# limeorange1102/multimodal-av-model

Hardware: AMD Instinct MI355X
Metric: utterances/sec (4 s clip, 25 fps 96x96 lip) at batch 64, full training step (higher is better)
Workload: dtype bf16; 1 GPU; BASELINE metric configuration (= configs[3]'s per-GPU batch): batch 64/GPU x 4 s (T_audio 64000, T_enc 199, 100 lip frames 96x96 x 2 speakers), wav2vec2-large + ResNet-18 + fusion BiLSTM + CTC + contrastive, fwd+bwd+Adam, random-init weights; variant=as_executed, global_batch=64, parallelism=dp1, audio_passes=2, wav2vec2_regularizers=hf-defaults (dropout 0.1, LayerDrop 0.1, SpecAugment 0.05)

## Files before the change

include/av_hip.h:

```cpp
#ifndef AV_HIP_H
#define AV_HIP_H
#ifdef __cplusplus
extern "C" {
#endif

#define AV_OK 0
#define AV_ERR_ARG 1
#define AV_ERR_LAUNCH 2

#define AV_F32 0
#define AV_BF16 1

#define AV_A_ROWMAJOR 0
#define AV_A_TRANS 1
#define AV_A_CONV2D 2
#define AV_A_CONV3D1 3
#define AV_B_NK 0
#define AV_B_KN 1
#define AV_ACT_NONE 0
#define AV_ACT_GELU 1
#define AV_ACT_MUL_GELU_GRAD 2
#define AV_ACT_GELU_GF 3
#define AV_ACT_MUL_AUX 4

// ... 61 lines not shown
                     int Tk, int D, long long q_bs, long long q_rs, long long k_bs, long long k_rs, long long v_bs,
                     long long v_rs, long long o_bs, long long o_rs, const int* klen, float scale, float drop_p,
                     unsigned long long drop_seed, unsigned int drop_stream, void* stream);
int av_attention_bwd(const void* q, const void* k, const void* v, const void* o, const void* dout, const float* lse,
                     float* delta_ws, void* dq, void* dk, void* dv, int B, int H, int Tq, int Tk, int D,
                     const long long* strides, const int* klen, float scale, float drop_p, unsigned long long drop_seed,
                     unsigned int drop_stream, void* stream);
int av_attention_dropmask(void* mask, int B, int H, int Tq, int Tk, float drop_p, unsigned long long drop_seed, unsigned int drop_stream,
                          void* stream);
int av_attention_fwd_mask(const void* q, const void* k, const void* v, void* o, float* lse, int dtype, int B, int H, int Tq,
                          int Tk, int D, long long q_bs, long long q_rs, long long k_bs, long long k_rs, long long v_bs,
                          long long v_rs, long long o_bs, long long o_rs, const int* klen, float scale, float drop_p,
                          unsigned long long drop_seed, unsigned int drop_stream, const void* drop_mask, void* stream);
int av_attention_bwd_mask(const void* q, const void* k, const void* v, const void* o, const void* dout, const float* lse,
                          float* delta_ws, void* dq, void* dk, void* dv, int B, int H, int Tq, int Tk, int D,
                          const long long* strides, const int* klen, float scale, float drop_p, unsigned long long drop_seed,
                          unsigned int drop_stream, const void* drop_mask, void* stream);
int av_softmax_rows(const float* s, void* p, int pdt, long long rows, int cols, float scale, const int* klen,
                    int rows_per_batch, int ld, void* stream);
int av_softmax_bwd_rows(const void* p, int pdt, const float* dp, void* ds, int dsdt, long long rows, int cols,
                        float scale, int ld, void* stream);

int av_conv0_ln_gelu(const float* wav, const float* w, const float* bias, const float* gamma, const float* beta, void* out,
                     int out_dtype, int B, int T_in, int L_out, int C, int k, int stride, float eps, void* stream);

int av_lstm_fwd_step(const float* gx, const void* whh, void* hseq, float* cseq, void* gates, void* out_bt, int dtype,
                     int T, int B, int H, int s, void* stream);
int av_lstm_bwd_step(const void* dout, int dout_dtype, long long do_bs, long long do_ts, void* dgates, const void* whhT,
                     const void* gates, const float* cseq, float* dc, int dtype, int T, int B, int H, int s, void* stream);

#define AV_LSTM_COUNTER_INTS 1024
int av_lstm_fwd_layer(const float* gx, const void* whh, void* hseq, float* cseq, void* gates, void* out_bt, int* counters,
                      int T, int B, int H, void* stream);
int av_lstm_bwd_layer(const void* dout, int dout_dtype, long long do_bs, long long do_ts, void* dgates, const void* whhT,
                      const void* gates, const float* cseq, float* dc, int* counters, int T, int B, int H, void* stream);

int av_mask_downsample(const long long* mask, long long* out, int B, int Tin, int Tout, void* stream);
int av_fusion_gather_lerp_fwd(const float* feat, const long long* mask, int* ws_i32, float* out, long long* mask_out,
                              long long* lens, int B, int Ta, int Tv, int D, int groups, void* stream);
int av_fusion_gather_lerp_bwd(const float* dout, const int* ws_i32, float* dfeat, int B, int Ta, int Tv, int D, int groups,
                              void* stream);
int av_permute_bt(const void* in, int idt, void* out, int odt, int B, int T, int D, void* stream);
int av_gather_rows(const void* src, int sdt, const long long* idx, void* out, int odt, long long n, int D, void* stream);
int av_scatter_rows(const float* src, const long long* idx, float* out, long long n, int D, float alpha, int accumulate,
                    void* stream);
int av_class_order(const long long* mask, long long n, long long* order, void* stream);

int av_conv3d_front(const float* x, const void* w, void* y, float* stats, int B, int T, int H, int W, void* stream);
int av_conv3d_front_pool(const float* x, const void* w, void* ymax, void* ymin, float* stats, int B, int T, int H, int W, void* stream);
int av_bn_prelu_minmax(const void* ymax, const void* ymin, const float* scale, const float* shift, const float* slope, void* out, long long n,
                       void* stream);
int av_conv3x3_c64(const void* x, const void* w, void* y, float* stats, int n_img, int H, int W, const float* in_scale,
                   const float* in_shift, const float* in_slope, void* stream);
int av_bn_finalize(const float* partial, int nblk, long long count, const float* gamma, const float* beta,
                   float* running_mean, float* running_var, float momentum, float eps, int training, float* scale,
                   float* shift, int C, double* ws, int ws_zeroed, void* stream);
int av_bn_act(const void* x, const float* scale, const float* shift, const void* res, const float* rscale,
              const float* rshift, const float* slope, void* out, int dtype, long long n, int C, void* stream);
int av_bn_prelu_maxpool(const void* x, const float* scale, const float* shift, const float* slope, void* out, int dtype,
                        long long N, int H, int W, int C, void* stream);
int av_avgpool(const void* x, int dtype, float* out, long long N, int HW, int C, int pm_block, void* stream);

int av_l2norm_fwd(const float* x, float* y, float* nrm, long long rows, int cols, float eps, void* stream);
int av_l2norm_bwd(const float* y, const float* dy, const float* nrm, float* dx, long long rows, int cols, float eps,
                  void* stream);
int av_lse_rows(const float* s, float* lse, float* rowsum, long long rows, int cols, int ld, void* stream);
int av_contrastive_dsim(const float* s, const float* lse, void* out, int odt, long long rows, int cols, int ld, float coef,
                        void* stream);
int av_lse_rows_chunk(const float* s, float* lse, float* rowsum, long long rows, int cols, int ld, int accumulate, void* stream);
int av_contrastive_dsim_chunk(const float* s, const float* lse, void* out, int odt, long long rows, int cols, int ld, float coef,
                              int total_cols, void* stream);
int av_reduce_sum(const float* x, long long n, float* out, float scale, int accumulate, void* stream);
int av_loss_combine(const float* nll, const float* w, const float* c1, const float* c2, float half_lambda, int n, float* out3,
                    void* stream);
int av_ctc_greedy(const float* log_probs, const long long* lengths, int* out_ids, int* out_len, int B, int T, int V, int blank,
                  void* stream);
int av_ctc_beam_workspace_bytes(int B, int T, int V, int beam_width, long long* bytes);
int av_ctc_beam_frame_pass(const float* log_probs, long long stride_b, long long stride_t, const long long* lengths, void* workspace,
                           long long workspace_bytes, int B, int T, int V, int blank, int beam_width, void* stream);
int av_ctc_beam_search(const float* log_probs, long long stride_b, long long stride_t, const long long* lengths, int* out_ids,
                       int* out_len, float* out_score, void* workspace, long long workspace_bytes, int B, int T, int V, int blank,
                       int beam_width, int nbest, void* stream);
int av_ctc_loss_fwd(const float* log_probs, long long stride_b, long long stride_t, const long long* targets, long long target_ld,
                    const long long* input_lengths, const long long* target_lengths, int B, int T, int V, int S_max, int blank,
                    int zero_infinity, float* nll, float* log_alpha, float* log_beta, void* stream);
int av_ctc_loss_bwd(const float* log_probs, long long stride_b, long long stride_t, const long long* targets, long long target_ld,
                    const long long* input_lengths, const long long* target_lengths, int B, int T, int V, int S_max, int blank,
                    const float* nll, const float* log_alpha, const float* log_beta, const float* grad_nll, float* grad, void* stream);
int av_lip_gray_resize(const void* src, int src_is_u8, float* dst, int T, int Hs, int Ws, int C, int Hd, int Wd, float divisor,
                       void* stream);
int av_mix_pair(const float* a1, long long len1, const float* a2, long long len2, float* mixed, long long* mask1, long long* mask2,
                unsigned* peak_ws, void* stream);
int av_adam_step(float* p, const float* g, float* m, float* v, long long n, float lr, float beta1, float beta2, float eps,
                 int step, float grad_scale, void* stream);
int av_adam_multi(const void* ptrs, const long long* sizes, const float* hyper, const int* chunk_tensor, const long long* chunk_start,
                  int n_chunks, int chunk_elems, int* steps, const int* step_slot, int n_tensors, float grad_scale,
                  float* scaler_state, float growth, float backoff, int growth_interval, void* stream);

int av_nchw_to_nhwc(const float* in, void* out, int out_dtype, long long N, int C, int H, int W, int Cp, void* stream);
int av_relu_maxpool2_fwd(const void* x, void* y, int dtype, long long N, int H, int W, int C, int nchw_out, void* stream);
int av_relu_maxpool2_bwd(const void* x, const void* dy, void* dx, int dtype, long long N, int H, int W, int C, int nchw_dy, void* stream);
int av_im2col3(const void* x, void* cols, int dtype, long long N, int H, int W, int C, void* stream);
int av_gru_fwd_step(const float* gx, const void* whh, const float* bhh, void* hseq, float* hf, float* gates, void* out_bt, int dtype,
                    int T, int B, int H, int s, void* stream);
int av_gru_bwd_step(const void* dout, int dout_dtype, long long do_bs, long long do_ts, void* dgi, void* dgh, const void* whhT,
                    const float* gates, const float* hf, float* dhc, int dtype, int T, int B, int H, int s, void* stream);
// ... 44 lines not shown
```

multimodal-av-model_amd/_lib.py:

```python
from __future__ import annotations

import ctypes as C
import os

from . import precision as _precision

_HERE = os.path.dirname(os.path.abspath(__file__))
LIB_PATH = os.environ.get("AVAMD_LIB") or os.path.join(_HERE, "libavhip.so")

AV_F32, AV_BF16 = 0, 1
A_ROWMAJOR, A_TRANS, A_CONV2D, A_CONV3D1 = 0, 1, 2, 3
B_NK, B_KN = 0, 1
ACT_NONE, ACT_GELU, ACT_MUL_GELU_GRAD, ACT_GELU_GF, ACT_MUL_AUX = 0, 1, 2, 3, 4
LSTM_COUNTER_INTS = 1024

vp, ll, i32, f32 = C.c_void_p, C.c_longlong, C.c_int, C.c_float


class GemmArgs(C.Structure):
    _fields_ = [
        ("A", vp), ("B", vp), ("C", vp), ("C2", vp), ("bias", vp), ("R", vp), ("aux", vp), ("stats", vp),
        ("M", i32), ("N", i32), ("K", i32), ("batch", i32),
        ("lda", ll), ("ldb", ll), ("ldc", ll), ("ldr", ll),
        ("sA", ll), ("sB", ll), ("sC", ll), ("sR", ll), ("sBias", ll),
        ("a_mode", i32), ("b_mode", i32), ("in_dtype", i32), ("out_dtype", i32), ("aux_dtype", i32), ("act", i32),
        ("alpha", f32),
        ("cT", i32), ("cH", i32), ("cW", i32), ("cCtot", i32), ("cCin", i32), ("cCoff", i32),
        ("cKt", i32), ("cKh", i32), ("cKw", i32), ("cSh", i32), ("cSw", i32), ("cPt", i32), ("cPh", i32), ("cPw", i32),
        ("cOh", i32), ("cOw", i32),
        ("batch_inner", i32), ("oA", ll), ("oB", ll), ("oC", ll),
        ("drop_p", f32), ("drop_stream", C.c_uint), ("drop_seed", C.c_ulonglong),
        ("k_total", i32), ("cNF", i32), ("cPM", i32),
    ]


class W2v2LayerArgs(C.Structure):
    _fields_ = [
        ("B", i32), ("T", i32), ("hidden", i32), ("heads", i32), ("inter", i32), ("lp", i32), ("gf", i32), ("stream_base", i32),
        ("eps", f32), ("scale", f32), ("hd_p", f32), ("at_p", f32), ("ac_p", f32),
        ("seed", C.c_ulonglong),
        ("ln1_g", vp), ("ln1_b", vp), ("ln2_g", vp), ("ln2_b", vp), ("b_qkv", vp), ("b_o", vp), ("b_1", vp), ("b_2", vp),
        ("w_qkv", vp), ("w_o", vp), ("w_1", vp), ("w_2", vp),
        ("h", vp), ("klen", vp), ("amask", vp),
        ("x1", vp), ("qkv", vp), ("ao", vp), ("x2", vp), ("u", vp), ("g", vp),
        ("mu1", vp), ("rs1", vp), ("lse", vp), ("h2", vp), ("mu2", vp), ("rs2", vp), ("h3", vp),
    ]


class W2v2LayerBwdArgs(C.Structure):
    _fields_ = [
        ("B", i32), ("T", i32), ("hidden", i32), ("heads", i32), ("inter", i32), ("lp", i32), ("gf", i32), ("stream_base", i32), ("lower_stream", i32),
        ("scale", f32), ("hd_p", f32), ("at_p", f32), ("ac_p", f32),
        ("seed", C.c_ulonglong),
        ("ln1_g", vp), ("ln2_g", vp),
        ("w_2t", vp), ("w_1t", vp), ("w_ot", vp), ("w_qkvt", vp),
        ("dh", vp), ("h", vp), ("mu1", vp), ("rs1", vp), ("lse", vp), ("h2", vp), ("mu2", vp), ("rs2", vp),
        ("dh_lp", vp), ("qkv", vp), ("ao", vp), ("amask", vp), ("u", vp),
        ("klen", vp),
        ("dh3_t", vp), ("du", vp), ("dx2", vp), ("dh2_lp", vp), ("dao", vp), ("dqkv", vp), ("dx1", vp), ("dh_out_lp", vp),
        ("dh2", vp), ("delta", vp), ("dh_out", vp),
    ]


SIGNATURES = {
    "av_last_error": [],
    "av_version": [],
    "av_gemm": [C.POINTER(GemmArgs), vp],
    "av_w2v2_layer_fwd": [C.POINTER(W2v2LayerArgs), vp],
    "av_w2v2_layer_bwd_dx": [C.POINTER(W2v2LayerBwdArgs), vp],
    "av_transpose": [vp, i32, vp, i32, i32, i32, ll, i32, vp],
    "av_sum_slices": [vp, i32, ll, ll, f32, vp, i32, vp],
    "av_layernorm_fwd": [vp, i32, vp, vp, vp, i32, vp, vp, ll, i32, f32, i32, vp],
    "av_layernorm_bwd_drop": [vp, i32, vp, i32, vp, vp, vp, vp, vp, vp, i32, ll, i32, vp, f32, C.c_ulonglong, C.c_uint, vp],
    "av_layernorm_bwd": [vp, i32, vp, i32, vp, vp, vp, vp, vp, vp, i32, ll, i32, vp, vp],
    "av_log_softmax_fwd": [vp, i32, vp, ll, i32, vp],
    "av_log_softmax_bwd": [vp, vp, vp, i32, ll, i32, vp],
    "av_log_softmax_bwd_ld": [vp, vp, vp, i32, ll, i32, i32, vp],
    "av_colsum": [vp, i32, vp, ll, i32, ll, i32, vp],
    "av_cast": [vp, i32, vp, i32, ll, vp],
    "av_cast_dropout": [vp, i32, vp, i32, ll, f32, C.c_ulonglong, C.c_uint, vp],
    "av_dropout_uniform": [vp, ll, C.c_ulonglong, C.c_uint, vp],
    "av_fusion_xattn_fwd": [vp, vp, vp, vp, vp, vp, vp, vp, i32, i32, i32, i32, f32, vp],
    "av_fusion_xattn_bwd": [vp, vp, vp, vp, vp, vp, vp, i32, i32, i32, i32, f32, vp],
    "av_zero_feature_cols": [vp, i32, vp, i32, i32, i32, vp],
    "av_overwrite_rows": [vp, i32, vp, vp, ll, i32, vp],
    "av_axpby": [f32, vp, i32, f32, vp, ll, vp],
    "av_mask_rows": [vp, i32, vp, ll, i32, vp],
    "av_mul_scalar_dev": [vp, vp, vp, ll, vp],
    "av_attention_fwd": [vp, vp, vp, vp, vp, i32, i32, i32, i32, i32, i32, ll, ll, ll, ll, ll, ll, ll, ll, vp, f32, f32, C.c_ulonglong, C.c_uint, vp],
    "av_attention_dropmask": [vp, i32, i32, i32, i32, f32, C.c_ulonglong, C.c_uint, vp],
    "av_attention_fwd_mask": [vp, vp, vp, vp, vp, i32, i32, i32, i32, i32, i32, ll, ll, ll, ll, ll, ll, ll, ll, vp, f32, f32, C.c_ulonglong, C.c_uint, vp, vp],
    "av_attention_bwd_mask": [vp, vp, vp, vp, vp, vp, vp, vp, vp, vp, i32, i32, i32, i32, i32, vp, vp, f32, f32, C.c_ulonglong, C.c_uint, vp, vp],
    "av_attention_bwd": [vp, vp, vp, vp, vp, vp, vp, vp, vp, vp, i32, i32, i32, i32, i32, vp, vp, f32, f32, C.c_ulonglong, C.c_uint, vp],
    "av_softmax_rows": [vp, vp, i32, ll, i32, f32, vp, i32, i32, vp],
    "av_conv0_ln_gelu": [vp, vp, vp, vp, vp, vp, i32, i32, i32, i32, i32, i32, i32, f32, vp],
    "av_lstm_fwd_step": [vp, vp, vp, vp, vp, vp, i32, i32, i32, i32, i32, vp],
    "av_lstm_bwd_step": [vp, i32, ll, ll, vp, vp, vp, vp, vp, i32, i32, i32, i32, i32, vp],
    "av_lstm_fwd_layer": [vp, vp, vp, vp, vp, vp, vp, i32, i32, i32, vp],
    "av_lstm_bwd_layer": [vp, i32, ll, ll, vp, vp, vp, vp, vp, vp, i32, i32, i32, vp],
    "av_mask_downsample": [vp, vp, i32, i32, i32, vp],
    "av_fusion_gather_lerp_fwd": [vp, vp, vp, vp, vp, vp, i32, i32, i32, i32, i32, vp],
    "av_fusion_gather_lerp_bwd": [vp, vp, vp, i32, i32, i32, i32, i32, vp],
    "av_permute_bt": [vp, i32, vp, i32, i32, i32, i32, vp],
    "av_gather_rows": [vp, i32, vp, vp, i32, ll, i32, vp],
    "av_scatter_rows": [vp, vp, vp, ll, i32, f32, i32, vp],
    "av_class_order": [vp, ll, vp, vp],
    "av_conv3d_front": [vp, vp, vp, vp, i32, i32, i32, i32, vp],
    "av_conv3d_front_pool": [vp, vp, vp, vp, vp, i32, i32, i32, i32, vp],
    "av_bn_prelu_minmax": [vp, vp, vp, vp, vp, vp, ll, vp],
    "av_conv3x3_c64": [vp, vp, vp, vp, i32, i32, i32, vp, vp, vp, vp],
    "av_bn_finalize": [vp, i32, ll, vp, vp, vp, vp, f32, f32, i32, vp, vp, i32, vp, i32, vp],
    "av_bn_act": [vp, vp, vp, vp, vp, vp, vp, vp, i32, ll, i32, vp],
    "av_bn_prelu_maxpool": [vp, vp, vp, vp, vp, i32, ll, i32, i32, i32, vp],
    "av_avgpool": [vp, i32, vp, ll, i32, i32, i32, vp],
    "av_l2norm_fwd": [vp, vp, vp, ll, i32, f32, vp],
    "av_l2norm_bwd": [vp, vp, vp, vp, ll, i32, f32, vp],
    "av_lse_rows": [vp, vp, vp, ll, i32, i32, vp],
    "av_lse_rows_chunk": [vp, vp, vp, ll, i32, i32, i32, vp],
    "av_contrastive_dsim_chunk": [vp, vp, vp, i32, ll, i32, i32, f32, i32, vp],
    "av_contrastive_dsim": [vp, vp, vp, i32, ll, i32, i32, f32, vp],
    "av_reduce_sum": [vp, ll, vp, f32, i32, vp],
    "av_loss_combine": [vp, vp, vp, vp, f32, i32, vp, vp],
    "av_ctc_greedy": [vp, vp, vp, vp, i32, i32, i32, i32, vp],
    "av_ctc_beam_workspace_bytes": [i32, i32, i32, i32, C.POINTER(ll)],
    "av_ctc_beam_frame_pass": [vp, ll, ll, vp, vp, ll, i32, i32, i32, i32, i32, vp],
    "av_ctc_beam_search": [vp, ll, ll, vp, vp, vp, vp, vp, ll, i32, i32, i32, i32, i32, i32, vp],
    "av_ctc_loss_fwd": [vp, ll, ll, vp, ll, vp, vp, i32, i32, i32, i32, i32, i32, vp, vp, vp, vp],
    "av_ctc_loss_bwd": [vp, ll, ll, vp, ll, vp, vp, i32, i32, i32, i32, i32, vp, vp, vp, vp, vp, vp],
    "av_lip_gray_resize": [vp, i32, vp, i32, i32, i32, i32, i32, i32, f32, vp],
    "av_mix_pair": [vp, ll, vp, ll, vp, vp, vp, vp, vp],
    "av_adam_multi": [vp, vp, vp, vp, vp, i32, i32, vp, vp, i32, f32, vp, f32, f32, i32, vp],
    "av_adam_step": [vp, vp, vp, vp, ll, f32, f32, f32, f32, i32, f32, vp],
    "av_softmax_bwd_rows": [vp, i32, vp, vp, i32, ll, i32, f32, i32, vp],
    "av_nchw_to_nhwc": [vp, vp, i32, ll, i32, i32, i32, i32, vp],
    "av_relu_maxpool2_fwd": [vp, vp, i32, ll, i32, i32, i32, i32, vp],
    "av_relu_maxpool2_bwd": [vp, vp, vp, i32, ll, i32, i32, i32, i32, vp],
    "av_im2col3": [vp, vp, i32, ll, i32, i32, i32, vp],
    "av_gru_fwd_step": [vp, vp, vp, vp, vp, vp, vp, i32, i32, i32, i32, i32, vp],
    "av_gru_bwd_step": [vp, i32, ll, ll, vp, vp, vp, vp, vp, vp, i32, i32, i32, i32, i32, vp],
    "av_wav_info": [C.c_char_p, C.POINTER(i32), C.POINTER(i32), C.POINTER(ll), C.POINTER(i32), C.POINTER(i32)],
    "av_wav_read_mono_f32": [C.c_char_p, ll, ll, vp],
    "av_resample_sinc": [vp, ll, vp, ll, vp, vp, i32, i32, i32, i32, vp],
}
_RESTYPES = {"av_last_error": C.c_char_p}

_libs = {}
_by_mode = {}


def _path() -> str:
    if _precision.get_precision() == "fp16":
        return os.environ.get("AVAMD_LIB_F16") or os.path.join(_HERE, "libavhip_f16.so")
    return LIB_PATH


def lib() -> C.CDLL:
    l = _by_mode.get(_precision._mode)
    if l is not None:
        return l
    path = _path()
    l = _libs.get(path)
    if l is None:
        if not os.path.exists(path):
# ... 19 lines not shown
```

multimodal-av-model_amd/model/encoder.py:

```python
from __future__ import annotations

import os
from typing import Optional, Union

import torch
import torch.nn as nn

from ..utils import init as _init
from .w2v2 import Wav2Vec2ModelHIP, load_local_config, load_local_weights, w2v2_apply


class AudioEncoder(nn.Module):

    def __init__(self, model_name: Union[str, dict] = "kresnik/wav2vec2-large-xlsr-korean", freeze: bool = True, seed: int = 2,
                 random_init: bool = False):
        super().__init__()
        weights = None
        if isinstance(model_name, dict):
            cfg = model_name
        elif os.path.isdir(model_name):
            cfg = load_local_config(model_name)
            weights = load_local_weights(model_name)
            if weights is None and not random_init:
                raise FileNotFoundError(
                    f"AudioEncoder: {model_name!r} holds neither model.safetensors nor pytorch_model.bin; training would start from an "
                    "untrained wav2vec2 — pass random_init=True if that is intended")
        else:
            raise FileNotFoundError(
                f"AudioEncoder: {model_name!r} is not a local directory; pretrained checkpoints cannot be fetched "
                "(no network) — pass a local HF wav2vec2 directory or a config dict")
        self.model = Wav2Vec2ModelHIP(cfg)
        if weights is not None and not cfg.get("conv_bias", True):
            for i, c in enumerate(cfg["conv_dim"]):
                weights.setdefault(f"feature_extractor.conv_layers.{i}.conv.bias", torch.zeros(c))
        sd = _init.w2v2_state_dict(cfg, seed=seed, prefix="") if weights is None else weights
        res = self.model.load_state_dict(sd, strict=False)
        if weights is not None:
            missing = [k for k in res.missing_keys if k != "masked_spec_embed"]
            if missing or res.unexpected_keys:
                raise KeyError(f"AudioEncoder: checkpoint does not match the architecture of config.json: missing {missing[:5]}, "
                               f"unexpected {list(res.unexpected_keys)[:5]}")
        self.output_dim = self.model.config.hidden_size
        if freeze:
            for p in self.model.parameters():
                p.requires_grad = False

    def forward(self, x: torch.Tensor, attention_mask: Optional[torch.Tensor] = None, valid_lengths=None):
        if not x.is_cuda:
            raise RuntimeError("AudioEncoder (HIP): input must be on the GPU; there is no CPU fallback")
        return w2v2_apply(self.model, x, attention_mask, valid_lengths=None if valid_lengths is None else (valid_lengths,))

    def forward_pair(self, x: torch.Tensor, attention_mask1: Optional[torch.Tensor], attention_mask2: Optional[torch.Tensor],
                     valid_lengths1=None, valid_lengths2=None):
        if not x.is_cuda:
            raise RuntimeError("AudioEncoder (HIP): input must be on the GPU; there is no CPU fallback")
        vl = None if valid_lengths1 is None or valid_lengths2 is None else (valid_lengths1, valid_lengths2)
        return w2v2_apply(self.model, x, attention_mask1, attention_mask2, two_passes=True, valid_lengths=vl)


from .. import _lib as L
from .. import ops
from ..precision import compute_dtype, is_lp

_TRUNK = ((64, 1), (128, 2), (256, 2), (512, 2))


FAST_C64 = os.environ.get("AVAMD_CONV_C64", "1") != "0"
FUSE_MID_ACT = os.environ.get("AVAMD_FUSE_MID_ACT", "1") != "0"
POS_MAJOR = os.environ.get("AVAMD_CONV_POSMAJOR", "1") != "0"
FRONT_POOL = os.environ.get("AVAMD_FRONT_POOL", "1") != "0"


class BasicBlock(nn.Module):

    def __init__(self, inplanes, planes, stride=1, downsample=None, relu_type="prelu"):
        super().__init__()
        if relu_type != "prelu":
            raise NotImplementedError("the HIP visual encoder implements relu_type='prelu' (what main.py:92 uses)")
        self.conv1 = nn.Conv2d(inplanes, planes, 3, stride, 1, bias=False)
        self.bn1 = nn.BatchNorm2d(planes)
        self.relu = nn.PReLU(planes)
        self.conv2 = nn.Conv2d(planes, planes, 3, 1, 1, bias=False)
        self.bn2 = nn.BatchNorm2d(planes)
        self.downsample = downsample
        self.stride = stride


class ResNet(nn.Module):
    def __init__(self, block=BasicBlock, layers=(2, 2, 2, 2), relu_type="prelu"):
        super().__init__()
        inpl = 64
        for li, ((planes, stride), nblk) in enumerate(zip(_TRUNK, layers), start=1):
            blocks = []
            for bi in range(nblk):
                st = stride if bi == 0 else 1
                ds = None
                if st != 1 or inpl != planes:
                    ds = nn.Sequential(nn.Conv2d(inpl, planes, 1, st, bias=False), nn.BatchNorm2d(planes))
                blocks.append(block(inpl, planes, st, ds, relu_type))
                inpl = planes
            setattr(self, f"layer{li}", nn.Sequential(*blocks))


class VisualEncoder(nn.Module):
    def __init__(self, relu_type="prelu"):
        super().__init__()
        if relu_type != "prelu":
            raise NotImplementedError("the HIP visual encoder implements relu_type='prelu'")
        self.frontend3D = nn.Sequential(
            nn.Conv3d(1, 64, kernel_size=(5, 7, 7), stride=(1, 2, 2), padding=(2, 3, 3), bias=False),
            nn.BatchNorm3d(64), nn.PReLU(64), nn.MaxPool3d((1, 3, 3), stride=(1, 2, 2), padding=(0, 1, 1)))
        self.trunk = ResNet(BasicBlock, [2, 2, 2, 2], relu_type=relu_type)
        self.output_dim = 512
        self._wcache = {}
        self._nbt = []
        self._bn_ws = None

    def _w(self, conv: nn.Module, dtype):
        p = conv.weight
        key = id(p)
        ver = (p._version, p.data_ptr(), dtype)
# ... 16 lines not shown
        if hit is None or hit[0] != ver:
            with torch.no_grad():
                w = torch.zeros((64, 36, 8), dtype=torch.float32, device=p.device)
                w[:, :35, :7] = p.data.reshape(64, 35, 7)
                hit = (ver, ops.cast(w.reshape(64, 288).contiguous(), compute_dtype()))
            self._wcache[key] = hit
        return hit[1]

    def warm_caches(self, dtype) -> None:
        conv0 = self.frontend3D[0]
        if is_lp(dtype) and tuple(conv0.kernel_size) == (5, 7, 7):
            self._w_front(conv0)
        self._w(conv0, dtype)
        for li in range(1, 5):
            for blk in getattr(self.trunk, f"layer{li}"):
                self._w(blk.conv1, dtype); self._w(blk.conv2, dtype)
                if blk.downsample is not None:
                    self._w(blk.downsample[0], dtype)

    def _bn(self, bn: nn.Module, stats, nblk: int, count: int, training: bool):
        C = bn.num_features
        dev = bn.weight.device
        scale = torch.empty(C, dtype=torch.float32, device=dev); shift = torch.empty(C, dtype=torch.float32, device=dev)
        ws = None
        if training:
            sid = ops.stream()
            if self._bn_ws is None or not isinstance(self._bn_ws, dict):
                self._bn_ws = {}
            ws = self._bn_ws.get(sid)
            if ws is None or ws.device != dev:
                ws = self._bn_ws[sid] = torch.zeros(2 * 1024, dtype=torch.float64, device=dev)
            sync = getattr(self, "_bn_sync", None)
            if sync is not None:
                mode, evs = sync
                i = self._bn_idx
                self._bn_idx += 1
                if mode == "follow" and i < len(evs):
                    torch.cuda.current_stream(dev).wait_event(evs[i])
        L.check(L.lib().av_bn_finalize(ops.ptr(stats), nblk, count, ops.ptr(bn.weight.data), ops.ptr(bn.bias.data),
                                       ops.ptr(bn.running_mean), ops.ptr(bn.running_var), float(bn.momentum), float(bn.eps),
                                       int(training), ops.ptr(scale), ops.ptr(shift), C, ops.ptr(ws), 1, ops.stream()), "av_bn_finalize")
        if training and getattr(self, "_bn_sync", None) is not None and self._bn_sync[0] == "lead":
            ev = torch.cuda.Event(); ev.record()
            self._bn_sync[1].append(ev)
        if training:
            self._nbt.append(bn.num_batches_tracked)
        return scale, shift

    def _c64_ok(self, conv: nn.Module, dtype, N, H, W, Cin) -> bool:
        k, st, pad = conv.kernel_size[0], conv.stride[0], conv.padding[0]
        return (is_lp(dtype) and (k, st, pad, Cin, conv.out_channels) == (3, 1, 1, 64, 64) and W <= 31
                and N * H * W < (1 << 24) and FAST_C64)

    def _conv2d(self, x, N, H, W, Cin, conv: nn.Module, dtype, training: bool, in_act=None, pm: int = 0):
        k, st = conv.kernel_size[0], conv.stride[0]
        pad = conv.padding[0]
        Cout = conv.out_channels
        Ho, Wo = (H + 2 * pad - k) // st + 1, (W + 2 * pad - k) // st + 1
        M = N * Ho * Wo
        y = torch.empty((M, Cout), dtype=dtype, device=x.device)
        if self._c64_ok(conv, dtype, N, H, W, Cin):
            nblk = (M + 255) // 256
            stats = torch.empty((nblk, 2, Cout), dtype=torch.float32, device=x.device) if training else None
            isc, ish, isl = in_act if in_act is not None else (None, None, None)
            L.check(L.lib().av_conv3x3_c64(ops.ptr(x), ops.ptr(self._w(conv, dtype)), ops.ptr(y), ops.ptr(stats), N, H, W,
                                           ops.ptr(isc), ops.ptr(ish), ops.ptr(isl), ops.stream()), "av_conv3x3_c64")
            return y, stats, nblk, M, Ho, Wo
        assert in_act is None
        nblk = (M + 127) // 128
        stats = torch.empty((nblk, 2, Cout), dtype=torch.float32, device=x.device) if training else None
        geo = dict(cT=1, cH=H, cW=W, cCtot=Cin, cCin=Cin, cCoff=0, cKt=1, cKh=k, cKw=k, cSh=st, cSw=st, cPt=0, cPh=pad, cPw=pad,
                   cOh=Ho, cOw=Wo, cNF=256 if pm else 0, cPM=pm)
        ops.gemm(x, self._w(conv, dtype), y, M=M, N=Cout, K=k * k * Cin, lda=0, ldb=k * k * Cin, ldc=Cout, a_mode=L.A_CONV2D,
                 conv=geo, stats=stats)
        return y, stats, nblk, M, Ho, Wo

    def _act(self, x, scale, shift, slope, res=None, rscale=None, rshift=None):
        out = torch.empty_like(x)
        L.check(L.lib().av_bn_act(ops.ptr(x), ops.ptr(scale), ops.ptr(shift), ops.ptr(res), ops.ptr(rscale), ops.ptr(rshift),
                                  ops.ptr(slope), ops.ptr(out), ops.dt(x), x.numel(), x.shape[-1], ops.stream()), "av_bn_act")
        return out

    @torch.no_grad()
    def _forward_impl(self, x: torch.Tensor) -> torch.Tensor:
        self._nbt = []
        if isinstance(self._bn_ws, dict) and x.is_cuda:
            ws = self._bn_ws.get(ops.stream())
            if ws is not None:
                ws.zero_()
        dtype = compute_dtype()
        training = self.training
        B, C, T, H, W = x.shape
        assert C == 1
        dev = x.device
        conv0 = self.frontend3D[0]
        kt, kh, kw = conv0.kernel_size
        Ho, Wo = (H + 2 * conv0.padding[1] - kh) // conv0.stride[1] + 1, (W + 2 * conv0.padding[2] - kw) // conv0.stride[2] + 1
        M = B * T * Ho * Wo
        fast = (is_lp(dtype) and (kt, kh, kw) == (5, 7, 7) and tuple(conv0.stride) == (1, 2, 2)
                and tuple(conv0.padding) == (2, 3, 3) and H % 16 == 0 and W % 32 == 0)
        N = B * T
        Hp, Wp = (Ho - 1) // 2 + 1, (Wo - 1) // 2 + 1
        pooled = None
        if fast and FRONT_POOL:
            nblk = B * T * (Ho // 8) * (Wo // 16)
            stats = torch.empty((nblk, 2, 64), dtype=torch.float32, device=dev) if training else None
            pooled = torch.empty((2, N * Hp * Wp, 64), dtype=dtype, device=dev)
            L.check(L.lib().av_conv3d_front_pool(ops.ptr(x.contiguous().float()), ops.ptr(self._w_front(conv0)), ops.ptr(pooled[0]), ops.ptr(pooled[1]),
                                                 ops.ptr(stats), B, T, H, W, ops.stream()), "av_conv3d_front_pool")
        elif fast:
            y = torch.empty((M, 64), dtype=dtype, device=dev)
            nblk = B * T * (Ho // 8) * (Wo // 16)
            stats = torch.empty((nblk, 2, 64), dtype=torch.float32, device=dev) if training else None
            L.check(L.lib().av_conv3d_front(ops.ptr(x.contiguous().float()), ops.ptr(self._w_front(conv0)), ops.ptr(y), ops.ptr(stats),
                                            B, T, H, W, ops.stream()), "av_conv3d_front")
        else:
            y = torch.empty((M, 64), dtype=dtype, device=dev)
            xin = ops.cast(x.contiguous().float().view(B, T, H, W), dtype)
            nblk = (M + 127) // 128
            stats = torch.empty((nblk, 2, 64), dtype=torch.float32, device=dev) if training else None
            geo = dict(cT=T, cH=H, cW=W, cCtot=1, cCin=1, cCoff=0, cKt=kt, cKh=kh, cKw=kw, cSh=conv0.stride[1], cSw=conv0.stride[2],
                       cPt=conv0.padding[0], cPh=conv0.padding[1], cPw=conv0.padding[2], cOh=Ho, cOw=Wo)
            ops.gemm(xin, self._w(conv0, dtype), y, M=M, N=64, K=kt * kh * kw, lda=0, ldb=kt * kh * kw, ldc=64, a_mode=L.A_CONV3D1,
                     conv=geo, stats=stats)
        sc, sh = self._bn(self.frontend3D[1], stats, nblk, M, training)
        h = torch.empty((N * Hp * Wp, 64), dtype=dtype, device=dev)
        if pooled is not None:
            L.check(L.lib().av_bn_prelu_minmax(ops.ptr(pooled[0]), ops.ptr(pooled[1]), ops.ptr(sc), ops.ptr(sh), ops.ptr(self.frontend3D[2].weight.data),
                                               ops.ptr(h), h.numel(), ops.stream()), "av_bn_prelu_minmax")
        else:
            L.check(L.lib().av_bn_prelu_maxpool(ops.ptr(y), ops.ptr(sc), ops.ptr(sh), ops.ptr(self.frontend3D[2].weight.data), ops.ptr(h),
                                                ops.dt(h), N, Ho, Wo, 64, ops.stream()), "av_bn_prelu_maxpool")
        Hc, Wc, Cc = Hp, Wp, 64
        FB = 256
        use_pm = POS_MAJOR and is_lp(dtype) and N % FB == 0
        pm_in = 0
        for li in range(1, 5):
            for blk in getattr(self.trunk, f"layer{li}"):
                slope = blk.relu.weight.data
                pm_out = 1 if (use_pm and li >= 2) else 0
                pm1 = pm_in | (pm_out << 1)
                pm2 = pm_out * 3
                if pm_out:
                    c1, st1, nb1, M1, H1, W1 = self._conv2d(h, N, Hc, Wc, Cc, blk.conv1, dtype, training, pm=pm1)
                    s1, b1 = self._bn(blk.bn1, st1, nb1, M1, training)
                    a1 = self._act(c1, s1, b1, slope)
                    c2, st2, nb2, M2, _, _ = self._conv2d(a1, N, H1, W1, blk.conv1.out_channels, blk.conv2, dtype, training, pm=pm2)
                    s2, b2 = self._bn(blk.bn2, st2, nb2, M2, training)
                    if blk.downsample is not None:
                        cd, std, nbd, Md, _, _ = self._conv2d(h, N, Hc, Wc, Cc, blk.downsample[0], dtype, training, pm=pm1)
                        sd, bd = self._bn(blk.downsample[1], std, nbd, Md, training)
                        h = self._act(c2, s2, b2, slope, res=cd, rscale=sd, rshift=bd)
                    else:
                        assert pm_in == pm_out, "position-major trunk: an identity residual needs its input in the layer's pixel order"
                        h = self._act(c2, s2, b2, slope, res=h)
                    Hc, Wc, Cc = H1, W1, blk.conv1.out_channels
                    pm_in = 1
                    continue
                c1, st1, nb1, M1, H1, W1 = self._conv2d(h, N, Hc, Wc, Cc, blk.conv1, dtype, training)
                s1, b1 = self._bn(blk.bn1, st1, nb1, M1, training)
                if FUSE_MID_ACT and self._c64_ok(blk.conv2, dtype, N, H1, W1, blk.conv1.out_channels):
                    c2, st2, nb2, M2, _, _ = self._conv2d(c1, N, H1, W1, blk.conv1.out_channels, blk.conv2, dtype, training,
                                                          in_act=(s1, b1, slope))
                else:
                    a1 = self._act(c1, s1, b1, slope)
                    c2, st2, nb2, M2, _, _ = self._conv2d(a1, N, H1, W1, blk.conv1.out_channels, blk.conv2, dtype, training)
                s2, b2 = self._bn(blk.bn2, st2, nb2, M2, training)
                if blk.downsample is not None:
                    cd, std, nbd, Md, _, _ = self._conv2d(h, N, Hc, Wc, Cc, blk.downsample[0], dtype, training)
                    sd, bd = self._bn(blk.downsample[1], std, nbd, Md, training)
                    h = self._act(c2, s2, b2, slope, res=cd, rscale=sd, rshift=bd)
                else:
                    h = self._act(c2, s2, b2, slope, res=h)
                Hc, Wc, Cc = H1, W1, blk.conv1.out_channels
        if self._nbt:
            torch._foreach_add_(self._nbt, 1)
            self._nbt = []
        out = torch.empty((N, Cc), dtype=torch.float32, device=dev)
        L.check(L.lib().av_avgpool(ops.ptr(h), ops.dt(h), ops.ptr(out), N, Hc * Wc, Cc, FB if pm_in else 0, ops.stream()), "av_avgpool")
        return out.view(B, T, Cc)

    def forward(self, x):
        if not x.is_cuda:
            raise RuntimeError("VisualEncoder (HIP): input must be on the GPU; there is no CPU fallback")
        if torch.is_grad_enabled() and any(p.requires_grad for p in self.parameters()):
            raise NotImplementedError("the HIP visual encoder is forward-only: freeze trunk and frontend3D as main.py:100-103 does")
        return self._forward_impl(x)
```

multimodal-av-model_amd/ops.py:

```python
from __future__ import annotations

import ctypes as C
import os
from typing import Optional

import torch

from . import _lib as L
from . import precision
from ._lib import AV_BF16, AV_F32

Tensor = torch.Tensor


def _lp() -> torch.dtype:
    return torch.float16 if precision.get_precision() == "fp16" else torch.bfloat16


def dt(t: Tensor) -> int:
    if t.dtype == torch.float32:
        return AV_F32
    if t.dtype == _lp():
        return AV_BF16
    raise TypeError(f"unsupported dtype {t.dtype} (the library of precision mode {precision.get_precision()!r} handles float32 / {_lp()})")
# ... 280 lines not shown
                                              ptr(part), nblk, rows, cols, ptr(dxl), float(lp_drop[0]), int(lp_drop[1]), int(lp_drop[2]), stream()),
                "av_layernorm_bwd_drop")
    else:
        L.check(L.lib().av_layernorm_bwd(ptr(x), dt(x), ptr(dy), dt(dy), ptr(gamma), ptr(mean), ptr(rstd), ptr(dres), ptr(dx),
                                         ptr(part), nblk, rows, cols, ptr(dxl), stream()), "av_layernorm_bwd")
    res = (dx,)
    if want_param_grads:
        if gb_acc is not None:
            gb = colsum(part, out=gb_acc, accumulate=True)
            res = (dx, gb)
        elif packed_gb:
            res = (dx, colsum(part))
        else:
            gb = colsum(part)
            res = (dx, gb[:cols], gb[cols:])
    if lp_copy:
        return res + (dxl,)
    return res if want_param_grads else dx


def log_softmax_fwd(x: Tensor) -> Tensor:
    cols = x.shape[-1]
    y = torch.empty(x.shape, dtype=torch.float32, device=x.device)
    L.check(L.lib().av_log_softmax_fwd(ptr(x), dt(x), ptr(y), x.numel() // cols, cols, stream()), "av_log_softmax_fwd")
    return y


def log_softmax_bwd(y: Tensor, dy: Tensor, out_dtype: torch.dtype, pad_to: int = 0) -> Tensor:
    cols = y.shape[-1]
    ldx = (cols + pad_to - 1) // pad_to * pad_to if pad_to > 0 else cols
    dx = torch.empty(y.shape[:-1] + (ldx,), dtype=out_dtype, device=y.device)
    L.check(L.lib().av_log_softmax_bwd_ld(ptr(y), ptr(dy), ptr(dx), dt(dx), y.numel() // cols, cols, ldx, stream()), "av_log_softmax_bwd")
    return dx


def colsum(x: Tensor, out: Optional[Tensor] = None, accumulate: bool = False) -> Tensor:
    cols = x.shape[-1]
    if x.is_contiguous():
        rows, ld = x.numel() // cols, cols
    else:
        assert x.dim() == 2 and x.stride(1) == 1
        rows, ld = x.shape[0], x.stride(0)
    if out is None:
        out = torch.empty(cols, dtype=torch.float32, device=x.device)
        accumulate = False
    L.check(L.lib().av_colsum(ptr(x), dt(x), ptr(out), rows, cols, ld, int(accumulate), stream()), "av_colsum")
    return out


def colsum_into(x: Tensor, zeroed_view: Optional[Tensor]) -> Tensor:
    return colsum(x, out=zeroed_view, accumulate=True) if zeroed_view is not None else colsum(x)


def cast(x: Tensor, dtype: torch.dtype) -> Tensor:
    if x.dtype == dtype:
        return x
    assert x.is_contiguous()
    y = torch.empty(x.shape, dtype=dtype, device=x.device)
    L.check(L.lib().av_cast(ptr(x), dt(x), ptr(y), dt(y), x.numel(), stream()), "av_cast")
    return y


def cast_dropout(x: Tensor, dtype: torch.dtype, drop: Optional[tuple]) -> Tensor:
    if drop is None or drop[0] <= 0:
        return cast(x, dtype)
    assert x.is_contiguous()
    y = torch.empty(x.shape, dtype=dtype, device=x.device)
    L.check(L.lib().av_cast_dropout(ptr(x), dt(x), ptr(y), dt(y), x.numel(), float(drop[0]), int(drop[1]), int(drop[2]), stream()), "av_cast_dropout")
    return y


def axpby(a: float, x: Tensor, b: float, y: Tensor) -> Tensor:
    assert x.is_contiguous() and y.is_contiguous() and y.dtype == torch.float32 and x.numel() == y.numel()
    L.check(L.lib().av_axpby(a, ptr(x), dt(x), b, ptr(y), x.numel(), stream()), "av_axpby")
    return y


def mask_rows_(x: Tensor, keep_u8: Tensor) -> Tensor:
    cols = x.shape[-1]
    L.check(L.lib().av_mask_rows(ptr(x), dt(x), ptr(keep_u8), x.numel() // cols, cols, stream()), "av_mask_rows")
    return x


def _chk_view(t: Tensor, name: str):
    if t.dim() != 4 or t.stride(3) != 1 or t.stride(2) != t.shape[3]:
        raise ValueError(f"{name}: expected a [B,T,H,D] view with contiguous D and head stride D, got {tuple(t.shape)} / {t.stride()}")


_ATTN_SHORT = os.environ.get("AVAMD_ATTN_SHORT", "1") != "0"


def attention_mask_shape_ok(dtype, B: int, Tq: int, Tk: int, D: int) -> bool:
    return _ATTN_SHORT and precision.is_lp(dtype) and D == 64 and Tq <= 256 and Tk <= 256 and B <= 65535


def attention_dropmask(B: int, H: int, Tq: int, Tk: int, drop: tuple, device) -> Tensor:
    mask = torch.empty((B, H, (Tq + 15) // 16, 64), dtype=torch.int64, device=device)
    L.check(L.lib().av_attention_dropmask(ptr(mask), B, H, Tq, Tk, float(drop[0]), int(drop[1]), int(drop[2]), stream()), "av_attention_dropmask")
    return mask


def attention_fwd(q: Tensor, k: Tensor, v: Tensor, klen: Optional[Tensor], scale: float, need_lse: bool = True,
                  drop: Optional[tuple] = None, drop_mask: Optional[Tensor] = None):
    for t, n in ((q, "q"), (k, "k"), (v, "v")):
        _chk_view(t, n)
    B, Tq, H, D = q.shape
# ... 162 lines not shown
```

Before: 989.8 utterances/s.

## Add windowed LDS 3x3 conv kernel for 128-channel ResNet layers with fused input activation

Adds a persistent HIP kernel for 3x3 stride-1 128->128 channel convolutions. It stages a window of whole images (up to 320 pixels) in LDS once and double-buffers the per-tap weight slices, instead of going through the generic implicit-GEMM path. It fuses the preceding BN+PReLU into the input load and computes per-tile BN statistics in the epilogue. It also stops using the position-major layout for blocks that take this path and routes conv2 through the fused mid-activation. This should cut global traffic and launches for ResNet layer2's conv2, but adds a large hand-scheduled kernel with tight LDS and register use.

After: 1002 utterances/s, median of 6. +1.2%, better.

```diff
diff --git a/include/av_hip.h b/include/av_hip.h
--- a/include/av_hip.h
+++ b/include/av_hip.h
@@ -137,6 +137,9 @@
                        void* stream);
 int av_conv3x3_c64(const void* x, const void* w, void* y, float* stats, int n_img, int H, int W, const float* in_scale,
                    const float* in_shift, const float* in_slope, void* stream);
+#define AV_CONV_C128_ROWS 320
+int av_conv3x3_c128(const void* x, const void* w, void* y, float* stats, int n_img, int H, int W, const float* in_scale,
+                    const float* in_shift, const float* in_slope, void* stream);
 int av_bn_finalize(const float* partial, int nblk, long long count, const float* gamma, const float* beta,
                    float* running_mean, float* running_var, float momentum, float eps, int training, float* scale,
                    float* shift, int C, double* ws, int ws_zeroed, void* stream);
diff --git a/multimodal-av-model_amd/_lib.py b/multimodal-av-model_amd/_lib.py
--- a/multimodal-av-model_amd/_lib.py
+++ b/multimodal-av-model_amd/_lib.py
@@ -12,6 +12,7 @@
 A_ROWMAJOR, A_TRANS, A_CONV2D, A_CONV3D1 = 0, 1, 2, 3
 B_NK, B_KN = 0, 1
 ACT_NONE, ACT_GELU, ACT_MUL_GELU_GRAD, ACT_GELU_GF, ACT_MUL_AUX = 0, 1, 2, 3, 4
+CONV_C128_ROWS = 320
 LSTM_COUNTER_INTS = 1024
 
 vp, ll, i32, f32 = C.c_void_p, C.c_longlong, C.c_int, C.c_float
@@ -109,6 +110,7 @@
     "av_conv3d_front_pool": [vp, vp, vp, vp, vp, i32, i32, i32, i32, vp],
     "av_bn_prelu_minmax": [vp, vp, vp, vp, vp, vp, ll, vp],
     "av_conv3x3_c64": [vp, vp, vp, vp, i32, i32, i32, vp, vp, vp, vp],
+    "av_conv3x3_c128": [vp, vp, vp, vp, i32, i32, i32, vp, vp, vp, vp],
     "av_bn_finalize": [vp, i32, ll, vp, vp, vp, vp, f32, f32, i32, vp, vp, i32, vp, i32, vp],
     "av_bn_act": [vp, vp, vp, vp, vp, vp, vp, vp, i32, ll, i32, vp],
     "av_bn_prelu_maxpool": [vp, vp, vp, vp, vp, i32, ll, i32, i32, i32, vp],
diff --git a/multimodal-av-model_amd/csrc/conv_window.hip b/multimodal-av-model_amd/csrc/conv_window.hip
--- /dev/null
+++ b/multimodal-av-model_amd/csrc/conv_window.hip
@@ -0,0 +1,296 @@
+#include <type_traits>
+
+#include "av_common.h"
+
+namespace {
+
+constexpr int WROWS = AV_CONV_C128_ROWS;
+constexpr int MAXPT = 5;
+constexpr int SLICE_BYTES = 128 * 256;
+constexpr int WIN_BYTES = WROWS * 256;
+constexpr int ST_BYTES = 4 * 2 * 128 * 4;
+constexpr int XP_BYTES = 3 * 128 * 4;
+constexpr int LDS_TOTAL = 2 * SLICE_BYTES + WIN_BYTES + ST_BYTES + XP_BYTES;
+
+typedef const __attribute__((address_space(1))) void* gptr_t;
+typedef __attribute__((address_space(3))) void* lptr_t;
+
+__device__ __forceinline__ void wg_barrier() {
+    asm volatile("" ::: "memory");
+    __builtin_amdgcn_s_waitcnt(0xC07F);
+    __builtin_amdgcn_s_barrier();
+    asm volatile("" ::: "memory");
+}
+
+__device__ __forceinline__ float row16_sum(float v) {
+    v += __builtin_bit_cast(float, __builtin_amdgcn_update_dpp(0, __builtin_bit_cast(int, v), 0x111, 0xf, 0xf, true));
+    v += __builtin_bit_cast(float, __builtin_amdgcn_update_dpp(0, __builtin_bit_cast(int, v), 0x112, 0xf, 0xf, true));
+    v += __builtin_bit_cast(float, __builtin_amdgcn_update_dpp(0, __builtin_bit_cast(int, v), 0x114, 0xf, 0xf, true));
+    v += __builtin_bit_cast(float, __builtin_amdgcn_update_dpp(0, __builtin_bit_cast(int, v), 0x118, 0xf, 0xf, true));
+    return v;
+}
+
+struct CP {
+    const bf16_t* x; const bf16_t* w; bf16_t* y; float* stats;
+    const float* in_scale; const float* in_shift; const float* in_slope;
+    int M, H, W, R, ntiles;
+};
+
+template <bool XF>
+__global__ __launch_bounds__(512) void conv3x3_c128_kernel(const CP p) {
+    extern __shared__ __attribute__((aligned(16))) char smem[];
+    char* Wl = smem;
+    char* win = smem + 2 * SLICE_BYTES;
+    float* St = (float*)(smem + 2 * SLICE_BYTES + WIN_BYTES);
+    float* Xp = (float*)(smem + 2 * SLICE_BYTES + WIN_BYTES + ST_BYTES);
+    const int tid = threadIdx.x, lane = tid & 63, w = __builtin_amdgcn_readfirstlane(tid >> 6);
+    const int r = lane & 15, g = lane >> 4;
+    const int wc = w & 1, wp = w >> 1;
+    const int G = gridDim.x;
+    if ((int)blockIdx.x >= p.ntiles) return;
+    const int T = (p.ntiles - (int)blockIdx.x + G - 1) / G;
+    const int PT = (p.R + 15) >> 4;
+    const int npt = (PT - wp + 3) >> 2;
+    const int ninstr = (p.R + 3) >> 2;
+    const int lrow = lane >> 4, lslot = lane & 15;
+
+    auto stage_w = [&](int tap, int slot, int k) {
+        const int ins = k * 8 + w;
+        const int n = ins * 4 + lrow;
+        const bf16_t* src = p.w + (long long)n * 1152 + tap * 128 + ((lslot ^ (n & 15)) << 3);
+        const unsigned off = __builtin_amdgcn_readfirstlane((unsigned)(slot * SLICE_BYTES + ins * 1024));
+        __builtin_amdgcn_global_load_lds((gptr_t)src, (lptr_t)(Wl + off), 16, 0, 0);
+    };
+    auto stage_x = [&](int tile, int ln) {
+        const int lrow = ln >> 4, lslot = ln & 15;
+        const long long q0 = (long long)tile * p.R;
+#pragma unroll
+        for (int k = 0; k < WROWS / 32; ++k) {
+            const int ins = k * 8 + w;
+            if (ins < ninstr) {
+                const int rl = ins * 4 + lrow;
+                long long q = q0 + rl;
+                q = q > p.M - 1 ? p.M - 1 : q;
+                const bf16_t* src = p.x + q * 128 + ((lslot ^ (rl & 15)) << 3);
+                const unsigned off = __builtin_amdgcn_readfirstlane((unsigned)(ins * 1024));
+                __builtin_amdgcn_global_load_lds((gptr_t)src, (lptr_t)(win + off), 16, 0, 0);
+            }
+        }
+    };
+#pragma unroll
+    for (int k = 0; k < 4; ++k) stage_w(0, 0, k);
+    stage_x((int)blockIdx.x, lane);
+    if constexpr (XF) {
+        if (tid < 128) { Xp[tid] = p.in_scale[tid]; Xp[128 + tid] = p.in_shift[tid]; Xp[256 + tid] = p.in_slope ? p.in_slope[tid] : 1.f; }
+    }
+    const int nst = p.R >> 5;
+
+    unsigned vm0[MAXPT];
+    int mrow[MAXPT];
+#pragma unroll
+    for (int i = 0; i < MAXPT; ++i) {
+        const int m = (i * 4 + wp) * 16 + r;
+        mrow[i] = m;
+        unsigned v = 0;
+        if (m < p.R) {
+            const int loc = m % (p.H * p.W);
+            const int yy = loc / p.W, xx = loc - yy * p.W;
+            v = (yy > 0 ? 1u : 0u) | 2u | (yy < p.H - 1 ? 4u : 0u) | (xx > 0 ? 8u : 0u) | 16u | (xx < p.W - 1 ? 32u : 0u);
+        }
+        vm0[i] = v;
+    }
+
+    int cnt = 0;
+    for (int t = 0; t < T; ++t) {
+        const int tile = (int)blockIdx.x + t * G;
+        const long long p0 = (long long)tile * p.R;
+        const int nvalid = p.M - p0 < p.R ? (int)(p.M - p0) : p.R;
+        const bool more = t + 1 < T;
+        if (t == 0) asm volatile("s_waitcnt vmcnt(0)" ::: "memory");
+        else if (nst >= 9) asm volatile("s_waitcnt vmcnt(9)" ::: "memory");
+        else asm volatile("s_waitcnt vmcnt(5)" ::: "memory");
+        wg_barrier();
+        if constexpr (XF) {
+            float xs[8], xb[8], xl[8];
+            {
+                const int cg = ((tid & 15) ^ ((tid >> 4) & 15)) * 8;
+#pragma unroll
+                for (int e = 0; e < 8; e += 4) {
+                    const f32x4 a = *(const f32x4*)(Xp + cg + e), b = *(const f32x4*)(Xp + 128 + cg + e), c = *(const f32x4*)(Xp + 256 + cg + e);
+#pragma unroll
+                    for (int q = 0; q < 4; ++q) { xs[e + q] = a[q]; xb[e + q] = b[q]; xl[e + q] = c[q]; }
+                }
+            }
+            uint4 tv[WROWS / 32];
+#pragma unroll
+            for (int k = 0; k < WROWS / 32; ++k) tv[k] = *(const uint4*)(win + (k * 512 + tid) * 16);
+#pragma unroll
+            for (int k = 0; k < WROWS / 32; ++k) {
+                const bf16x8 v = __builtin_bit_cast(bf16x8, tv[k]);
+                bf16x8 o;
+#pragma unroll
+                for (int e = 0; e < 8; ++e) {
+                    const float f = (float)v[e] * xs[e] + xb[e];
+                    o[e] = (bf16_t)(f >= 0.f ? f : f * xl[e]);
+                }
+                *(uint4*)(win + (k * 512 + tid) * 16) = __builtin_bit_cast(uint4, o);
+            }
+            wg_barrier();
+        }
+        auto body = [&](auto npt_c) __attribute__((always_inline)) {
+            constexpr int NPT = decltype(npt_c)::value;
+            f32x4 acc[4][NPT];
+#pragma unroll
+            for (int i = 0; i < NPT; ++i)
+#pragma unroll
+                for (int j = 0; j < 4; ++j) acc[j][i] = f32x4{0.f, 0.f, 0.f, 0.f};
+#pragma unroll 1
+            for (int tap = 0; tap < 9; ++tap, ++cnt) {
+                const int ky = tap / 3, kx = tap - ky * 3;
+                const unsigned wo = (unsigned)((cnt & 1) * SLICE_BYTES + (wc * 64 + r) * 256 + ((g ^ r) << 4));
+                const int nslot = (cnt + 1) & 1, ntap = tap == 8 ? 0 : tap + 1;
+                const bool pre = tap < 8 || more;
+                const int doff = (ky - 1) * p.W + (kx - 1);
+                unsigned pa[NPT];
+                bool ok[NPT];
+#pragma unroll
+                for (int i = 0; i < NPT; ++i) {
+                    int q = mrow[i] + doff;
+                    q = q < 0 ? 0 : (q > WROWS - 1 ? WROWS - 1 : q);
+                    pa[i] = (unsigned)(q * 256 + ((g ^ (q & 15)) << 4));
+                    ok[i] = ((vm0[i] >> ky) & 1u) && ((vm0[i] >> (3 + kx)) & 1u);
+                }
+                bf16x8 wfA[4], pfA[NPT], wfB[4], pfB[NPT];
+#define C128_LOAD(WF, PF, KS)                                                                                            \
+        {                                                                                                                    \
+            _Pragma("unroll") for (int j = 0; j < 4; ++j) WF[j] = *(const bf16x8*)(Wl + (wo ^ (unsigned)((KS) << 6)) + j * 4096); \
+            _Pragma("unroll") for (int i = 0; i < NPT; ++i)                                                                \
+                PF[i] = *(const bf16x8*)(win + (pa[i] ^ (unsigned)((KS) << 6)));                                 \
+        }
+#define C128_MMA(WF, PF)                                                                                                 \
+        {                                                                                                                    \
+            _Pragma("unroll") for (int i = 0; i < NPT; ++i)                                                                \
+            {                                                                                                                \
+                if (!ok[i]) PF[i] = bf16x8{0, 0, 0, 0, 0, 0, 0, 0};                                                          \
+                _Pragma("unroll") for (int j = 0; j < 4; ++j)                                                                \
+                    acc[j][i] = AV_MFMA_F32_16X16X32_LP(WF[j], PF[i], acc[j][i], 0, 0, 0);                                   \
+            }                                                                                                                \
+        }
+                C128_LOAD(wfA, pfA, 0)
+#pragma unroll
+                for (int ks = 0; ks < 4; ks += 2) {
+                    __builtin_amdgcn_s_waitcnt(0xC07F);
+                    C128_LOAD(wfB, pfB, ks + 1)
+                    __builtin_amdgcn_sched_barrier(0);
+                    C128_MMA(wfA, pfA)
+                    if (pre && ks == 0) { stage_w(ntap, nslot, 0); stage_w(ntap, nslot, 1); }
+                    __builtin_amdgcn_sched_barrier(0);
+                    __builtin_amdgcn_s_waitcnt(0xC07F);
+                    if (ks + 2 < 4) C128_LOAD(wfA, pfA, ks + 2)
+                    __builtin_amdgcn_sched_barrier(0);
+                    C128_MMA(wfB, pfB)
+                    if (pre && ks == 0) { stage_w(ntap, nslot, 2); stage_w(ntap, nslot, 3); }
+                    __builtin_amdgcn_sched_barrier(0);
+                }
+#undef C128_LOAD
+#undef C128_MMA
+                asm volatile("s_waitcnt vmcnt(0)" ::: "memory");
+                wg_barrier();
+            }
+#pragma unroll
+            for (int i = 0; i < NPT; ++i)
+                {
+                    const int rl = mrow[i];
+#pragma unroll
+                    for (int j = 0; j < 4; ++j) {
+                        bf16x4 o;
+#pragma unroll
+                        for (int e = 0; e < 4; ++e) o[e] = (bf16_t)acc[j][i][e];
+                        *(bf16x4*)(win + rl * 256 + (((wc * 8 + 2 * j + (g >> 1)) ^ (rl & 15)) << 4) + 8 * (g & 1)) = o;
+                    }
+                }
+            if (p.stats) {
+#pragma unroll
+                for (int j = 0; j < 4; ++j)
+#pragma unroll
+                    for (int e = 0; e < 4; ++e) {
+                        float s1 = 0.f, s2 = 0.f;
+#pragma unroll
+                        for (int i = 0; i < NPT; ++i) {
+                            const float v = mrow[i] < nvalid ? acc[j][i][e] : 0.f;
+                            s1 += v; s2 += v * v;
+                        }
+                        s1 = row16_sum(s1); s2 = row16_sum(s2);
+                        if (r == 15) {
+                            St[(wp * 2 + 0) * 128 + wc * 64 + j * 16 + 4 * g + e] = s1;
+                            St[(wp * 2 + 1) * 128 + wc * 64 + j * 16 + 4 * g + e] = s2;
+                        }
+                    }
+            }
+        };
+        switch (npt) {
+            case 5: body(std::integral_constant<int, 5>{}); break;
+            case 4: body(std::integral_constant<int, 4>{}); break;
+            case 3: body(std::integral_constant<int, 3>{}); break;
+            default: body(std::integral_constant<int, 2>{}); break;
+        }
+        wg_barrier();
+        {
+            uint4 ov[WROWS / 32];
+            int tq = tid;
+            asm volatile("" : "+v"(tq));
+#pragma unroll
+            for (int k = 0; k < WROWS / 32; ++k) {
+                const int id = k * 512 + tq, rl = id >> 4, ch = id & 15;
+                ov[k] = *(const uint4*)(win + rl * 256 + ((ch ^ (rl & 15)) << 4));
+            }
+            float sv = 0.f;
+            if (p.stats && tid < 256) {
+                const int which = tid >> 7, c = tid & 127;
+                sv = St[(0 * 2 + which) * 128 + c] + St[(1 * 2 + which) * 128 + c] + St[(2 * 2 + which) * 128 + c] + St[(3 * 2 + which) * 128 + c];
+            }
+            wg_barrier();
+            if (more) stage_x(tile + G, tq & 63);
+#pragma unroll
+            for (int k = 0; k < WROWS / 32; ++k) asm volatile("" :: "v"(ov[k].x), "v"(ov[k].y), "v"(ov[k].z), "v"(ov[k].w));
+#pragma unroll
+            for (int k = 0; k < WROWS / 32; ++k) {
+                const int id = k * 512 + tq, rl = id >> 4, ch = id & 15;
+                if (rl < nvalid) *(uint4*)(p.y + (p0 + rl) * 128 + ch * 8) = ov[k];
+            }
+            if (p.stats && tid < 256) p.stats[(long long)tile * 256 + tid] = sv;
+        }
+    }
+}
+
+}
+
+extern "C" int av_conv3x3_c128(const void* x, const void* w, void* y, float* stats, int n_img, int H, int W, const float* in_scale,
+                               const float* in_shift, const float* in_slope, void* stream) {
+    AV_CHECK(x && w && y, "av_conv3x3_c128: null pointer");
+    AV_CHECK((in_scale == nullptr) == (in_shift == nullptr) && (in_scale || !in_slope), "av_conv3x3_c128: in_scale / in_shift come together");
+    AV_CHECK(n_img > 0 && H > 0 && W > 0 && (long long)H * W <= WROWS && (long long)n_img * H * W < (1ll << 24),
+             "av_conv3x3_c128: bad shape n=%d H=%d W=%d (H*W <= %d, n*H*W < 2^24)", n_img, H, W, WROWS);
+    AV_CHECK((uintptr_t)x % 16 == 0 && (uintptr_t)w % 16 == 0 && (uintptr_t)y % 16 == 0, "av_conv3x3_c128: operands must be 16-byte aligned");
+    static int ncu = 0;
+    if (!ncu) {
+        int dev = 0;
+        if (hipGetDevice(&dev) != hipSuccess || hipDeviceGetAttribute(&ncu, hipDeviceAttributeMultiprocessorCount, dev) != hipSuccess || ncu <= 0) ncu = 256;
+        if (hipFuncSetAttribute((const void*)conv3x3_c128_kernel<false>, hipFuncAttributeMaxDynamicSharedMemorySize, LDS_TOTAL) != hipSuccess ||
+            hipFuncSetAttribute((const void*)conv3x3_c128_kernel<true>, hipFuncAttributeMaxDynamicSharedMemorySize, LDS_TOTAL) != hipSuccess) {
+            ncu = 0;
+            av_set_error("av_conv3x3_c128: cannot raise dynamic LDS to %d", LDS_TOTAL);
+            return AV_ERR_LAUNCH;
+        }
+    }
+    CP p;
+    p.x = (const bf16_t*)x; p.w = (const bf16_t*)w; p.y = (bf16_t*)y; p.stats = stats;
+    p.in_scale = in_scale; p.in_shift = in_shift; p.in_slope = in_slope;
+    const int ipt = WROWS / (H * W);
+    p.M = n_img * H * W; p.H = H; p.W = W; p.R = ipt * H * W; p.ntiles = (n_img + ipt - 1) / ipt;
+    const int G = p.ntiles < ncu ? p.ntiles : ncu;
+    if (in_scale) hipLaunchKernelGGL(conv3x3_c128_kernel<true>, dim3(G), dim3(512), LDS_TOTAL, (hipStream_t)stream, p);
+    else hipLaunchKernelGGL(conv3x3_c128_kernel<false>, dim3(G), dim3(512), LDS_TOTAL, (hipStream_t)stream, p);
+    AV_LAUNCH_CHECK();
+    return AV_OK;
+}
diff --git a/multimodal-av-model_amd/model/encoder.py b/multimodal-av-model_amd/model/encoder.py
--- a/multimodal-av-model_amd/model/encoder.py
+++ b/multimodal-av-model_amd/model/encoder.py
@@ -67,6 +67,7 @@
 
 FAST_C64 = os.environ.get("AVAMD_CONV_C64", "1") != "0"
 FUSE_MID_ACT = os.environ.get("AVAMD_FUSE_MID_ACT", "1") != "0"
+FAST_C128 = os.environ.get("AVAMD_CONV_C128", "1") != "0"
 POS_MAJOR = os.environ.get("AVAMD_CONV_POSMAJOR", "1") != "0"
 FRONT_POOL = os.environ.get("AVAMD_FRONT_POOL", "1") != "0"
 
@@ -189,6 +190,11 @@
         return (is_lp(dtype) and (k, st, pad, Cin, conv.out_channels) == (3, 1, 1, 64, 64) and W <= 31
                 and N * H * W < (1 << 24) and FAST_C64)
 
+    def _c128_ok(self, conv: nn.Module, dtype, N, H, W, Cin) -> bool:
+        k, st, pad = conv.kernel_size[0], conv.stride[0], conv.padding[0]
+        return (is_lp(dtype) and (k, st, pad, Cin, conv.out_channels) == (3, 1, 1, 128, 128) and H * W <= L.CONV_C128_ROWS
+                and N * H * W < (1 << 24) and FAST_C128)
+
     def _conv2d(self, x, N, H, W, Cin, conv: nn.Module, dtype, training: bool, in_act=None, pm: int = 0):
         k, st = conv.kernel_size[0], conv.stride[0]
         pad = conv.padding[0]
@@ -202,6 +208,14 @@
             isc, ish, isl = in_act if in_act is not None else (None, None, None)
             L.check(L.lib().av_conv3x3_c64(ops.ptr(x), ops.ptr(self._w(conv, dtype)), ops.ptr(y), ops.ptr(stats), N, H, W,
                                            ops.ptr(isc), ops.ptr(ish), ops.ptr(isl), ops.stream()), "av_conv3x3_c64")
+            return y, stats, nblk, M, Ho, Wo
+        if pm == 0 and self._c128_ok(conv, dtype, N, H, W, Cin):
+            ipt = L.CONV_C128_ROWS // (H * W)
+            nblk = (N + ipt - 1) // ipt
+            stats = torch.empty((nblk, 2, Cout), dtype=torch.float32, device=x.device) if training else None
+            isc, ish, isl = in_act if in_act is not None else (None, None, None)
+            L.check(L.lib().av_conv3x3_c128(ops.ptr(x), ops.ptr(self._w(conv, dtype)), ops.ptr(y), ops.ptr(stats), N, H, W,
+                                            ops.ptr(isc), ops.ptr(ish), ops.ptr(isl), ops.stream()), "av_conv3x3_c128")
             return y, stats, nblk, M, Ho, Wo
         assert in_act is None
         nblk = (M + 127) // 128
@@ -275,7 +289,10 @@
         for li in range(1, 5):
             for blk in getattr(self.trunk, f"layer{li}"):
                 slope = blk.relu.weight.data
-                pm_out = 1 if (use_pm and li >= 2) else 0
+                c1c = blk.conv1
+                Hn, Wn = (Hc + 2 * c1c.padding[0] - c1c.kernel_size[0]) // c1c.stride[0] + 1, (Wc + 2 * c1c.padding[0] - c1c.kernel_size[0]) // c1c.stride[0] + 1
+                win = self._c128_ok(blk.conv2, dtype, N, Hn, Wn, c1c.out_channels)
+                pm_out = 1 if (use_pm and li >= 2 and not win) else 0
                 pm1 = pm_in | (pm_out << 1)
                 pm2 = pm_out * 3
                 if pm_out:
@@ -296,7 +313,8 @@
                     continue
                 c1, st1, nb1, M1, H1, W1 = self._conv2d(h, N, Hc, Wc, Cc, blk.conv1, dtype, training)
                 s1, b1 = self._bn(blk.bn1, st1, nb1, M1, training)
-                if FUSE_MID_ACT and self._c64_ok(blk.conv2, dtype, N, H1, W1, blk.conv1.out_channels):
+                if FUSE_MID_ACT and (self._c64_ok(blk.conv2, dtype, N, H1, W1, blk.conv1.out_channels)
+                                     or self._c128_ok(blk.conv2, dtype, N, H1, W1, blk.conv1.out_channels)):
                     c2, st2, nb2, M2, _, _ = self._conv2d(c1, N, H1, W1, blk.conv1.out_channels, blk.conv2, dtype, training,
                                                           in_act=(s1, b1, slope))
                 else:
diff --git a/multimodal-av-model_amd/ops.py b/multimodal-av-model_amd/ops.py
--- a/multimodal-av-model_amd/ops.py
+++ b/multimodal-av-model_amd/ops.py
@@ -356,6 +356,19 @@
     return colsum(x, out=zeroed_view, accumulate=True) if zeroed_view is not None else colsum(x)
 
 
+def conv3x3_c128(x: Tensor, wk: Tensor, n_img: int, H: int, W: int, *, stats: bool = True, in_act: Optional[tuple] = None):
+    _req(x, "x"); _req(wk, "wk")
+    ipt = L.CONV_C128_ROWS // (H * W) if H * W <= L.CONV_C128_ROWS else 0
+    if ipt == 0:
+        raise ValueError(f"conv3x3_c128: H * W = {H * W} exceeds the {L.CONV_C128_ROWS}-pixel window")
+    nblk = (n_img + ipt - 1) // ipt
+    y = torch.empty((n_img * H * W, 128), dtype=x.dtype, device=x.device)
+    st = torch.empty((nblk, 2, 128), dtype=torch.float32, device=x.device) if stats else None
+    isc, ish, isl = in_act if in_act is not None else (None, None, None)
+    L.check(L.lib().av_conv3x3_c128(ptr(x), ptr(wk), ptr(y), ptr(st), n_img, H, W, ptr(isc), ptr(ish), ptr(isl), stream()), "av_conv3x3_c128")
+    return y, st, nblk
+
+
 def cast(x: Tensor, dtype: torch.dtype) -> Tensor:
     if x.dtype == dtype:
         return x
```
